# ehgus8/alpha-zero

Hardware: AMD Instinct MI355X
Metric: selfplay_games_per_sec (higher is better)
Workload: dtype bf16

## Files before the change

### alpha-zero_amd/azk/__init__.py

```python
import ctypes as C
import math
import os
import subprocess

import numpy as np

_HERE = os.path.dirname(os.path.abspath(__file__))
_CSRC = os.path.join(os.path.dirname(_HERE), "csrc")
LIB_PATH = os.path.join(_HERE, "libazk.so")

ABI_VERSION = 4
GAME_ID = {"tictactoe": 0, "connect4": 1, "gomoku": 2}
LEAF_F32, LEAF_BF16 = 0, 1
EMBED_POOL_COMPACT_MAX_SLOTS = 65279

SYMBOLS = [
    "azk_abi_version", "azk_last_error", "azk_create", "azk_destroy", "azk_geometry", "azk_reset_games",
    "azk_set_positions", "azk_begin_search", "azk_step_select", "azk_step_expand_backup", "azk_step",
    "azk_root_stats", "azk_root_children", "azk_export_tree", "azk_advance", "azk_get_positions",
    "azk_get_counters", "azk_reset_counters", "azk_check_device_error", "azk_gen_noise",
    "azk_rules_legal_moves", "azk_rules_legal_mask", "azk_rules_apply_move", "azk_rules_undo_move",
    "azk_rules_check_winner", "azk_rules_canonical", "azk_softmax_rows",
    "azk_step_tree", "azk_step_gather", "azk_recycle_finished", "azk_nn_patch_embed", "azk_nn_cls_attention", "azk_nn_patch_embed_scores", "azk_nn_cls_pool", "azk_debug_stamps", "azk_debug_stamps_raw", "azk_emit_finished", "azk_clear_cache", "azk_nn_heads_finalize", "azk_nn_layernorm_rows",
    "azk_vanilla_set_rng", "azk_vanilla_get_rng", "azk_vanilla_search", "azk_nn_embed_pool",
    "azk_nn_gemm_rows", "azk_nn_layernorm_sum", "azk_nn_heads_finalize_sum", "azk_nn_ln_heads",
    "azk_leaf_source_of", "azk_nn_embed_pool_leaves", "azk_nn_embed_pool_compact", "azk_nn_embed_pool_compact_leaves",
    "azk_nn_embed_fold", "azk_nn_embed_fold_leaves", "azk_nnx_embed_fold", "azk_nnx_embed_fold_leaves",
    "azk_nn_tail_gemm", "azk_nn_tail_gemm_lds", "azk_nn_tail_lds_footprint", "azk_nn_embed_fold_grid", "azk_nn_gemm_tok", "azk_nn_attention_tok", "azk_begin_search_budget", "azk_search_unfinished",
    "azk_nnx_embed_pool", "azk_nnx_embed_pool_leaves", "azk_nnx_gemm", "azk_nnx_gemm_h", "azk_nnx_gemm_h_lds",
    "azk_async_begin", "azk_async_step", "azk_async_drain", "azk_async_set_budget",
]


class AzkError(RuntimeError):
    pass


class Config(C.Structure):
    _fields_ = [("game", C.c_int32), ("rows", C.c_int32), ("cols", C.c_int32), ("n_games", C.c_int32),
                ("max_sims", C.c_int32), ("leaf_dtype", C.c_int32), ("device", C.c_int32),
                ("arena_nodes", C.c_int32), ("cache_entries", C.c_int32), ("cache_shared", C.c_int32), ("leaves_per_step", C.c_int32),
                ("tree_reuse", C.c_int32), ("reserved", C.c_int32 * 4)]


class LeafSource(C.Structure):
    _fields_ = [("leaf_flag", C.c_void_p), ("leaf_cells", C.c_void_p), ("to_move", C.c_void_p), ("leaf_depth", C.c_void_p),
                ("leaf_slot", C.c_void_p), ("n_leaf", C.c_void_p), ("n_games", C.c_int32), ("rows", C.c_int32), ("cols", C.c_int32),
                ("rc", C.c_int32), ("rc_pad", C.c_int32), ("planes", C.c_int32), ("flag_bytes", C.c_int32), ("cache_stamp", C.c_void_p)]


class EmbedPoolConsts(C.Structure):
    _fields_ = [("wt_frag", C.c_void_p), ("cpos_tok", C.c_void_p), ("score_tok", C.c_void_p), ("wconst_tok", C.c_void_p),
                ("xnconst_tok", C.c_void_p), ("z_all", C.c_void_p), ("l_all", C.c_void_p), ("score_msum", C.c_void_p),
                ("score_ref", C.c_void_p), ("num_heads", C.c_int32), ("ksize", C.c_int32), ("kp", C.c_int32),
                ("embed_dim", C.c_int32), ("ln_eps", C.c_float), ("work_stats", C.c_void_p)]


class EmbedFoldConsts(C.Structure):
    _fields_ = [("g_frag", C.c_void_p), ("e_frag", C.c_void_p), ("u2_tok", C.c_void_p), ("score_tok", C.c_void_p),
                ("wconst_tok", C.c_void_p), ("l_all", C.c_void_p), ("score_ref", C.c_void_p), ("inv_scales", C.c_void_p),
                ("num_heads", C.c_int32), ("ksize", C.c_int32), ("embed_dim", C.c_int32), ("ln_eps", C.c_float),
                ("work_stats", C.c_void_p)]


class TailGemm(C.Structure):
    _fields_ = [("a_bf16", C.c_void_p), ("lda", C.c_int32), ("a_batch_stride", C.c_int32), ("w_packed", C.c_void_p),
                ("m", C.c_int32), ("n_out", C.c_int32), ("k", C.c_int32), ("nbatch", C.c_int32), ("n_valid", C.c_void_p),
                ("bias", C.c_void_p), ("layernorm_a", C.c_int32), ("epilogue", C.c_int32), ("ln_eps", C.c_float),
                ("a_stats", C.c_void_p), ("a_stats_groups", C.c_int32), ("stats_out", C.c_void_p),
                ("out_bf16", C.c_void_p), ("ldo", C.c_int32), ("resid_bf16", C.c_void_p), ("ldr", C.c_int32),
                ("logits_out", C.c_void_p), ("values_out", C.c_void_p), ("action_dim", C.c_int32), ("a_col_sums", C.c_void_p)]


class GemmTok(C.Structure):
    _fields_ = [("a_bf16", C.c_void_p), ("lda", C.c_int32), ("w_packed", C.c_void_p), ("m", C.c_int32), ("n_out", C.c_int32), ("k", C.c_int32),
                ("n_valid", C.c_void_p), ("bias", C.c_void_p), ("epilogue", C.c_int32), ("out", C.c_void_p), ("ldo", C.c_int32),
                ("resid_bf16", C.c_void_p), ("ldr", C.c_int32)]


class EmbedPoolXConsts(C.Structure):
    _fields_ = [("wt_frag", C.c_void_p), ("cpos_tok", C.c_void_p), ("score_tok", C.c_void_p), ("wconst_tok", C.c_void_p),
                ("xnconst_tok", C.c_void_p), ("z_all", C.c_void_p), ("l_all", C.c_void_p), ("score_msum", C.c_void_p),
                ("score_ref", C.c_void_p), ("num_heads", C.c_int32), ("ksize", C.c_int32), ("kp", C.c_int32),
                ("embed_dim", C.c_int32), ("ln_eps", C.c_float), ("wt_scale", C.c_float), ("work_stats", C.c_void_p),
                ("wconst_h16_tok", C.c_void_p), ("pool_scale", C.c_float)]


class GemmX(C.Structure):
    _fields_ = [("a_f32", C.c_void_p), ("lda", C.c_int32), ("a_batch_stride", C.c_int32), ("w_packed", C.c_void_p),
                ("m", C.c_int32), ("n_out", C.c_int32), ("k", C.c_int32), ("nbatch", C.c_int32), ("n_valid", C.c_void_p),
                ("bias", C.c_void_p), ("layernorm_a", C.c_int32), ("epilogue", C.c_int32), ("ln_eps", C.c_float),
                ("a_stats", C.c_void_p), ("stats_out", C.c_void_p), ("out_f32", C.c_void_p), ("ldo", C.c_int32),
                ("resid_f32", C.c_void_p), ("ldr", C.c_int32), ("logits_out", C.c_void_p), ("values_out", C.c_void_p),
                ("action_dim", C.c_int32)]


class GemmH(C.Structure):
    _fields_ = [("a_hi", C.c_void_p), ("a_lo", C.c_void_p), ("a_f32", C.c_void_p), ("lda", C.c_int32), ("a_batch_stride", C.c_int32),
                ("w_packed", C.c_void_p), ("m", C.c_int32), ("n_out", C.c_int32), ("k", C.c_int32), ("nbatch", C.c_int32),
                ("n_valid", C.c_void_p), ("bias", C.c_void_p), ("col_sums", C.c_void_p), ("layernorm_a", C.c_int32), ("epilogue", C.c_int32),
                ("ln_eps", C.c_float), ("a_scale", C.c_float), ("w_scale", C.c_float), ("a_stats", C.c_void_p), ("stats_out", C.c_void_p),
                ("out_hi", C.c_void_p), ("out_lo", C.c_void_p), ("out_f32", C.c_void_p), ("ldo", C.c_int32), ("resid_f32", C.c_void_p),
                ("ldr", C.c_int32), ("logits_out", C.c_void_p), ("values_out", C.c_void_p), ("action_dim", C.c_int32), ("overflow_flag", C.c_void_p)]

# ... 64 lines not shown
    L.azk_clear_cache.argtypes = [vp, vp]
    L.azk_emit_finished.argtypes = [vp, vp, vp, vp, i64, vp, vp, vp]
    L.azk_debug_stamps.argtypes = [vp, vp]
    L.azk_check_device_error.argtypes = [vp, vp]
    L.azk_gen_noise.argtypes = [vp, u64, i64, i32, f64, vp, vp, vp]
    for name in ("azk_rules_legal_moves",):
        getattr(L, name).argtypes = [i32, i32, i32, vp, i32, vp, vp, vp]
    L.azk_rules_legal_mask.argtypes = [i32, i32, i32, vp, i32, vp, vp]
    L.azk_rules_apply_move.argtypes = [i32, i32, i32, vp, i32, vp, vp, vp, vp]
    L.azk_rules_undo_move.argtypes = [i32, i32, i32, vp, i32, vp, vp, vp]
    L.azk_rules_check_winner.argtypes = [i32, i32, i32, vp, i32, vp, vp, vp, vp]
    L.azk_rules_canonical.argtypes = [i32, i32, i32, vp, i32, vp, vp, vp]
    L.azk_softmax_rows.argtypes = [vp, i32, i32, vp, vp]
    L.azk_step_tree.argtypes = [vp, vp, vp, vp]
    L.azk_vanilla_set_rng.argtypes = [vp, i32, i32, vp, vp]
    L.azk_vanilla_get_rng.argtypes = [vp, i32, i32, vp, vp]
    L.azk_vanilla_search.argtypes = [vp, i32, vp]
    L.azk_step_gather.argtypes = [vp, vp, vp, vp]
    L.azk_recycle_finished.argtypes = [vp, vp, vp]
    L.azk_nn_patch_embed_scores.argtypes = [vp, i32, vp, vp, vp, vp, vp, vp, vp, vp, i32, i32, i32, i32, i32, i32, i32, i32, C.c_float, vp, vp]
    L.azk_nn_embed_pool.argtypes = [vp, i32, vp, vp, vp, vp, vp, vp, i32, i32, i32, i32, i32, i32, i32, i32, C.c_float, vp, vp]
    L.azk_leaf_source_of.argtypes = [vp, vp, C.POINTER(LeafSource)]
    L.azk_nn_embed_pool_leaves.argtypes = [C.POINTER(LeafSource), vp, vp, vp, vp, vp, vp, i32, i32, i32, i32, C.c_float, vp]
    L.azk_nn_embed_pool_compact.argtypes = [vp, i32, C.POINTER(EmbedPoolConsts), vp, i32, i32, i32, i32, vp, vp, vp]
    L.azk_nn_embed_pool_compact_leaves.argtypes = [C.POINTER(LeafSource), C.POINTER(EmbedPoolConsts), vp, vp, vp]
    L.azk_nn_embed_fold.argtypes = [vp, i32, C.POINTER(EmbedFoldConsts), vp, i32, i32, i32, i32, vp, vp, vp]
    L.azk_nn_embed_fold_leaves.argtypes = [C.POINTER(LeafSource), C.POINTER(EmbedFoldConsts), vp, vp, vp]
    L.azk_nnx_embed_fold.argtypes = [vp, i32, C.POINTER(EmbedFoldConsts), vp, i32, i32, i32, i32, vp, vp, vp]
    L.azk_nnx_embed_fold_leaves.argtypes = [C.POINTER(LeafSource), C.POINTER(EmbedFoldConsts), vp, vp, vp]
    L.azk_begin_search_budget.argtypes = [vp, vp, i32, i32, vp]
    L.azk_search_unfinished.argtypes = [vp, vp, vp]
    L.azk_nn_tail_gemm.argtypes = [C.POINTER(TailGemm), vp]
    L.azk_nn_tail_gemm_lds.argtypes = [C.POINTER(TailGemm), vp]
    L.azk_nn_gemm_tok.argtypes = [C.POINTER(GemmTok), vp]
    L.azk_nn_attention_tok.argtypes = [vp, vp, i32, i32, i32, i32, vp, vp]
    L.azk_nnx_embed_pool.argtypes = [vp, i32, C.POINTER(EmbedPoolXConsts), vp, i32, i32, i32, i32, vp, vp, vp]
    L.azk_nnx_embed_pool_leaves.argtypes = [C.POINTER(LeafSource), C.POINTER(EmbedPoolXConsts), vp, vp, vp]
    L.azk_nnx_gemm.argtypes = [C.POINTER(GemmX), vp]
    L.azk_nnx_gemm_h.argtypes = [C.POINTER(GemmH), vp]
    L.azk_nnx_gemm_h_lds.argtypes = [C.POINTER(GemmH), vp]
    L.azk_async_begin.argtypes = [vp, C.POINTER(AsyncConfig), vp]
    L.azk_async_step.argtypes = [vp, vp, vp, i32, vp]
    L.azk_async_set_budget.argtypes = [vp, i32, i32, vp]
    L.azk_async_drain.argtypes = [vp, vp, vp, vp, i64, vp, vp]
    L.azk_nn_ln_heads.argtypes = [vp, vp, vp, C.c_float, vp, vp, i32, i32, i32, i32, vp, vp, vp, vp]
    L.azk_nn_gemm_rows.argtypes = [vp, i32, vp, i32, i32, i32, i32, vp, vp, vp, vp, vp]
    L.azk_nn_layernorm_sum.argtypes = [vp, i32, i32, vp, vp, vp, vp, C.c_float, vp, vp, vp, i32, i32, vp, vp]
    L.azk_nn_heads_finalize_sum.argtypes = [vp, i32, i32, i32, vp, i32, i32, vp, vp, vp, vp]
    L.azk_nn_layernorm_rows.argtypes = [vp, vp, vp, C.c_float, vp, vp, i32, i32, vp, vp]
    L.azk_nn_heads_finalize.argtypes = [vp, i32, i32, i32, vp, vp, vp, vp]
    L.azk_nn_cls_pool.argtypes = [vp, vp, vp, vp, i32, i32, i32, i32, vp, vp]
    L.azk_nn_cls_attention.argtypes = [vp, vp, vp, i32, vp, i32, i32, i32, i32, vp]
    L.azk_nn_patch_embed.argtypes = [vp, i32, vp, vp, vp, vp, vp, vp, i32, i32, i32, i32, i32, i32, i32, C.c_float, vp]
    for name in SYMBOLS:
        f = getattr(L, name)
        if name not in ("azk_last_error", "azk_destroy"):
            f.restype = i32
    _LIB = L
    return L


def _torch():
    import torch
    if not torch.cuda.is_available():
        raise AzkError("no GPU visible: the azk engine runs only on an MI355X (no CPU fallback)")
    return torch
# ... 672 lines not shown

def nn_tail_gemm(a, w_packed, n_out, k, epilogue=TAIL_BF16, nbatch=1, a_batch_stride=0, bias=None, out=None, resid=None,
                 a_stats=None, stats_out=None, logits=None, values=None, action_dim=0, count=None, eps=1e-5, col_sums=None, lds=False):
    torch = _torch()
    assert a.dtype == torch.bfloat16 and a.stride(-1) == 1 and a.dim() == 2
    d = TailGemm()
    d.a_bf16, d.lda, d.a_batch_stride, d.w_packed = a.data_ptr(), a.stride(0), int(a_batch_stride), w_packed.data_ptr()
    d.m, d.n_out, d.k, d.nbatch = a.shape[0], int(n_out), int(k), int(nbatch)
    d.n_valid = count.data_ptr() if count is not None else None
    d.bias = bias.data_ptr() if bias is not None else None
    d.layernorm_a, d.epilogue, d.ln_eps = (1 if a_stats is not None else 0), int(epilogue), float(eps)
    if a_stats is not None:
        assert a_stats.dtype == torch.float32 and a_stats.dim() == 3 and a_stats.shape[2] == 2 and a_stats.is_contiguous()
        d.a_stats, d.a_stats_groups = a_stats.data_ptr(), a_stats.shape[1]
    if stats_out is not None:
        assert stats_out.dtype == torch.float32 and tuple(stats_out.shape) == (a.shape[0], nbatch * n_out // 64, 2) and stats_out.is_contiguous()
        d.stats_out = stats_out.data_ptr()
    if out is not None:
        assert out.dtype == torch.bfloat16 and out.stride(-1) == 1
        d.out_bf16, d.ldo = out.data_ptr(), out.stride(0)
    if resid is not None:
        d.resid_bf16, d.ldr = resid.data_ptr(), resid.stride(0)
    if logits is not None:
        assert logits.dtype == torch.float32 and values.dtype == torch.float32 and logits.is_contiguous()
        d.logits_out, d.values_out, d.action_dim = logits.data_ptr(), values.data_ptr(), int(action_dim)
    if col_sums is not None:
        assert col_sums.dtype == torch.float32 and col_sums.is_contiguous() and col_sums.numel() >= nbatch * n_out
        d.a_col_sums = col_sums.data_ptr()
    rc = (lib().azk_nn_tail_gemm_lds if lds else lib().azk_nn_tail_gemm)(C.byref(d), _stream())
    if rc != 0:
        raise AzkError(f"azk_nn_tail_gemm{'_lds' if lds else ''} failed ({rc})")


TOK_BF16, TOK_GELU, TOK_RESID, TOK_F32 = 0, 1, 2, 4


def pack_linear_weight128(w):
    torch = _torch()
    n_out, k = w.shape
    npad = (n_out + 127) // 128 * 128
    wp = torch.zeros(npad, k, dtype=torch.float32, device=w.device)
    wp[:n_out] = w.float()
    return pack_linear_weight(wp)


def nn_gemm_tok(a, w_packed, n_out, epilogue=TOK_BF16, bias=None, out=None, resid=None, count=None):
    torch = _torch()
    assert a.dtype == torch.bfloat16 and a.dim() == 2 and a.stride(1) == 1 and n_out % 128 == 0
    m, k = a.shape
    if out is None:
        out = torch.empty((m, n_out), dtype=torch.float32 if epilogue == TOK_F32 else torch.bfloat16, device=a.device)
    assert out.stride(1) == 1 and out.dtype == (torch.float32 if epilogue == TOK_F32 else torch.bfloat16)
    d = GemmTok()
    d.a_bf16, d.lda, d.w_packed, d.m, d.n_out, d.k = a.data_ptr(), a.stride(0), w_packed.data_ptr(), m, int(n_out), k
    d.n_valid = count.data_ptr() if count is not None else None
    if bias is not None:
        assert bias.dtype == torch.float32 and bias.numel() >= n_out
        d.bias = bias.data_ptr()
    d.epilogue, d.out, d.ldo = int(epilogue), out.data_ptr(), out.stride(0)
    if resid is not None:
        assert resid.dtype == torch.bfloat16 and resid.stride(1) == 1
        d.resid_bf16, d.ldr = resid.data_ptr(), resid.stride(0)
    rc = lib().azk_nn_gemm_tok(C.byref(d), _stream())
    if rc != 0:
        raise AzkError(f"azk_nn_gemm_tok failed ({rc})")
    return out
# ... 352 lines not shown
```

### alpha-zero_amd/csrc/azk_nn.hip

```cpp
#include <hip/hip_runtime.h>
#include <hip/hip_bf16.h>
#include <stdint.h>
#include <stdio.h>
#include <stdlib.h>
#include <string.h>
#include <type_traits>

#include "azk.h"
#include "azk_launch.h"
#include "azk_tail_common.h"

namespace {

typedef __attribute__((ext_vector_type(8))) __bf16 bf16x8;
typedef __attribute__((ext_vector_type(4))) float f32x4;

struct EmbedArgs {
    const void *boards;
    int boards_f32;
    const __hip_bfloat16 *wt;
    const float *cpos;
    const float *ln_w, *ln_b;
    __hip_bfloat16 *x;
    __hip_bfloat16 *xhat;
// ... 2540 lines not shown
        uint2 rr[EPI == TAIL_EPI_RESID ? RT : 1][4];
        if (EPI == TAIL_EPI_RESID) {
#pragma unroll
            for (int i = 0; i < RT; i++)
#pragma unroll
                for (int j = 0; j < 4; j++) rr[i][j] = *(const uint2 *)(a.resid + (size_t)min(row0 + 16 * i + 4 * l4 + j, a.M - 1) * a.ldr + col0);
        }
        if (EPI == TAIL_EPI_HEADS) {
            f32x4 hv[RT][4];
#pragma unroll
            for (int i = 0; i < RT; i++)
#pragma unroll
                for (int j = 0; j < 4; j++) {
                    hv[i][j] = f32x4{acc[i][0][j] + bv[0], acc[i][1][j] + bv[1], acc[i][2][j] + bv[2], acc[i][3][j] + bv[3]};
#pragma unroll
                    for (int c = 0; c < 4; c++)
                        if (col0 + c == a.action_dim) hv[i][j][c] = tanhf(hv[i][j][c]);
                }
#pragma unroll
            for (int i = 0; i < RT; i++)
#pragma unroll
                for (int j = 0; j < 4; j++) {
                    const int row = row0 + 16 * i + 4 * l4 + j;
#pragma unroll
                    for (int c = 0; c < 4; c++) {
                        const int col = col0 + c;
                        if (row < nvalid && col < a.action_dim) a.logits[(size_t)row * a.action_dim + col] = hv[i][j][c];
                        if (row < nvalid && col == a.action_dim) a.values[row] = hv[i][j][c];
                    }
                }
        } else {
            uint2 o[RT][4];
            f32x2 ps[RT][4];
#pragma unroll
            for (int i = 0; i < RT; i++)
#pragma unroll
                for (int j = 0; j < 4; j++) {
                    f32x4 v = {acc[i][0][j] + bv[0], acc[i][1][j] + bv[1], acc[i][2][j] + bv[2], acc[i][3][j] + bv[3]};
                    if (EPI == TAIL_EPI_GELU) {
#pragma unroll
                        for (int c = 0; c < 4; c++) v[c] = gelu_erf(v[c]);
                    }
                    if (EPI == TAIL_EPI_RESID) {
                        v[0] += __uint_as_float(rr[i][j].x << 16); v[1] += __uint_as_float(rr[i][j].x & 0xffff0000u);
                        v[2] += __uint_as_float(rr[i][j].y << 16); v[3] += __uint_as_float(rr[i][j].y & 0xffff0000u);
                    }
                    union { bf16x4 b4; uint2 u; } ob;
                    ob.b4 = __builtin_convertvector(v, bf16x4);
                    o[i][j] = ob.u;
                    if (a.stats_out) {
                        const f32x4 vr = __builtin_convertvector(ob.b4, f32x4);
                        ps[i][j] = f32x2{row16_sum((vr[0] + vr[1]) + (vr[2] + vr[3])),
                                         row16_sum((vr[0] * vr[0] + vr[1] * vr[1]) + (vr[2] * vr[2] + vr[3] * vr[3]))};
                    }
                }
            const int ngr = a.nbatch * (a.N >> 6), gr = b * (a.N >> 6) + g;
#pragma unroll
            for (int i = 0; i < RT; i++)
#pragma unroll
                for (int j = 0; j < 4; j++) {
                    const int row = row0 + 16 * i + 4 * l4 + j;
                    if (row < nvalid) *(uint2 *)(a.out + (size_t)row * a.ldo + col0) = o[i][j];
                    if (a.stats_out && l15 == 0 && row < nvalid) *(f32x2 *)(a.stats_out + ((size_t)row * ngr + gr) * 2) = ps[i][j];
                }
        }
    }
}

template <int RTLO, int RTHI, int KCH, int AMODE, int EPI, int NWR, int NWC, int NWK>
__global__ __launch_bounds__(64 * NWR * NWC * NWK, 1) void k_tail_gemm(TailArgs a) {
    __shared__ f32x4 kred[NWK > 1 ? (NWK - 1) * RTHI * 4 * 64 : 1];
    asm volatile("" :: "s"(a.A), "s"(a.Wp), "s"(a.out), "s"(a.bias), "s"(a.resid), "s"(a.stats_in), "s"(a.stats_out), "s"(a.logits), "s"(a.values),
                 "s"(a.lda), "s"(a.ldo), "s"(a.N), "s"(a.nbatch), "s"(a.wave_slots), "s"(a.M), "s"(a.a_batch), "s"(a.w_batch), "s"(a.ldr),
                 "s"(a.ln_eps), "s"(a.action_dim));
    const int nvalid = a.count ? min(a.M, *a.count) : a.M;
    const int strip_waves = (a.N >> 6) * a.nbatch * NWK;
    int rt = RTLO;
    while (rt < RTHI && ((nvalid + 16 * rt * NWR - 1) / (16 * rt * NWR)) * NWR * strip_waves > a.wave_slots) rt++;
    if (RTHI >= RTLO + 2 && rt == RTLO + 2) tail_items<(RTHI >= RTLO + 2 ? RTLO + 2 : RTLO), KCH, AMODE, EPI, NWR, NWC, NWK>(a, nvalid, kred);
    else if (RTHI >= RTLO + 1 && rt == RTLO + 1) tail_items<(RTHI >= RTLO + 1 ? RTLO + 1 : RTLO), KCH, AMODE, EPI, NWR, NWC, NWK>(a, nvalid, kred);
    else tail_items<RTLO, KCH, AMODE, EPI, NWR, NWC, NWK>(a, nvalid, kred);
}

int tail_cu_count() {
    static int cus = 0;
    if (!cus) {
        int dev = 0;
        if (hipGetDevice(&dev) != hipSuccess || hipDeviceGetAttribute(&cus, hipDeviceAttributeMultiprocessorCount, dev) != hipSuccess || cus <= 0) cus = 256;
    }
    return cus;
}

template <int RTLO, int RTHI, int KCH, int AMODE, int EPI, int NWR, int NWC, int NWK = 1>
int launch_tail(TailArgs &a, hipStream_t st) {
    static_assert(RTHI <= RTLO + 2, "three tile heights per kernel");
    static int slots = 0;
    if (!slots) {
        int nb = 0;
        if (hipOccupancyMaxActiveBlocksPerMultiprocessor(&nb, k_tail_gemm<RTLO, RTHI, KCH, AMODE, EPI, NWR, NWC, NWK>, 64 * NWR * NWC * NWK, 0) != hipSuccess || nb < 1) nb = 1;
        slots = nb * NWR * NWC * NWK * tail_cu_count();
    }
    a.wave_slots = slots;
    const long long items = (long long)((a.M + 16 * RTLO * NWR - 1) / (16 * RTLO * NWR)) * (a.N / (64 * NWC)) * a.nbatch;
    const unsigned blocks = (unsigned)(items < 8192 ? items : 8192);
    k_tail_gemm<RTLO, RTHI, KCH, AMODE, EPI, NWR, NWC, NWK><<<blocks, 64 * NWR * NWC * NWK, 0, st>>>(a);
    return hipGetLastError() == hipSuccess ? AZK_OK : AZK_ERR_HIP;
}
}

extern "C" int32_t azk_nn_tail_gemm(const azk_tail_gemm *t, void *stream) {
    if (!t || !t->a_bf16 || !t->w_packed || t->m < 0 || t->n_out < 64 || (t->n_out & 63) || t->nbatch < 1) return AZK_ERR_ARG;
    if ((t->k != 512 && t->k != 2048 && t->k != 384) || t->lda < t->k || (t->lda & 7) || (t->a_batch_stride & 7)) return AZK_ERR_ARG;
    if (t->epilogue < 0 || t->epilogue > 3 || (t->layernorm_a && (t->k != 512 || !t->a_stats || t->a_stats_groups != 8))) return AZK_ERR_ARG;
    if (t->epilogue == TAIL_EPI_HEADS ? (!t->logits_out || !t->values_out || t->action_dim + 1 > t->n_out * t->nbatch) : (!t->out_bf16 || t->ldo < t->n_out * t->nbatch || (t->ldo & 3)))
        return AZK_ERR_ARG;
    if (t->epilogue == TAIL_EPI_RESID && (!t->resid_bf16 || (t->ldr & 3))) return AZK_ERR_ARG;
    if (t->m == 0) return AZK_OK;
    TailArgs a = {};
    a.A = (const unsigned short *)t->a_bf16; a.lda = t->lda; a.a_batch = t->a_batch_stride; a.Wp = (const uint4 *)t->w_packed;
    a.w_batch = (long long)(t->n_out / 64) * (t->k / 32) * 4 * 64;
    a.M = t->m; a.N = t->n_out; a.nbatch = t->nbatch; a.count = t->n_valid; a.bias = t->bias; a.out = (unsigned short *)t->out_bf16; a.ldo = t->ldo;
    a.resid = (const unsigned short *)t->resid_bf16; a.ldr = t->ldr; a.ln_eps = t->ln_eps; a.logits = t->logits_out; a.values = t->values_out;
    a.action_dim = t->action_dim; a.stats_in = t->a_stats; a.stats_groups = t->a_stats_groups; a.stats_out = t->stats_out;
    hipStream_t st = (hipStream_t)stream;
    const bool wide = t->n_out % 128 == 0 && t->n_out >= 1024;
    if (t->k == 384)
        return !t->layernorm_a && t->epilogue == TAIL_EPI_BF16 ? launch_tail<2, 2, 3, 0, TAIL_EPI_BF16, 1, 1, 4>(a, st) : AZK_ERR_ARG;
    if (t->k == 512) {
        if (t->layernorm_a) {
            if (t->epilogue == TAIL_EPI_GELU) return wide ? launch_tail<2, 4, 16, 1, TAIL_EPI_GELU, 2, 2>(a, st) : launch_tail<2, 2, 16, 1, TAIL_EPI_GELU, 1, 1>(a, st);
            if (t->epilogue == TAIL_EPI_HEADS) return launch_tail<1, 1, 4, 1, TAIL_EPI_HEADS, 1, 1, 4>(a, st);
            if (t->epilogue == TAIL_EPI_BF16) return launch_tail<2, 2, 16, 1, TAIL_EPI_BF16, 1, 1>(a, st);
            return AZK_ERR_ARG;
        }
        if (t->epilogue == TAIL_EPI_BF16) return launch_tail<2, 2, 4, 0, TAIL_EPI_BF16, 1, 1, 4>(a, st);
        if (t->epilogue == TAIL_EPI_GELU) return wide ? launch_tail<2, 4, 16, 0, TAIL_EPI_GELU, 2, 2>(a, st) : launch_tail<2, 2, 16, 0, TAIL_EPI_GELU, 1, 1>(a, st);
        if (t->epilogue == TAIL_EPI_RESID) return launch_tail<2, 2, 16, 0, TAIL_EPI_RESID, 1, 1>(a, st);
        return launch_tail<2, 2, 16, 0, TAIL_EPI_HEADS, 1, 1>(a, st);
    }
    if (t->epilogue == TAIL_EPI_RESID) return launch_tail<2, 4, 16, 0, TAIL_EPI_RESID, 1, 1, 4>(a, st);
    if (t->epilogue == TAIL_EPI_BF16) return launch_tail<2, 4, 16, 0, TAIL_EPI_BF16, 1, 1, 4>(a, st);
    return AZK_ERR_ARG;
}
```

### alpha-zero_amd/csrc/azk_tail_common.h

```cpp
#pragma once
#include <hip/hip_runtime.h>
#include <stdint.h>

namespace azk_tail {

typedef __attribute__((ext_vector_type(8))) __bf16 bf16x8;
typedef __attribute__((ext_vector_type(4))) __bf16 bf16x4;
typedef __attribute__((ext_vector_type(4))) float f32x4;
typedef __attribute__((ext_vector_type(2))) float f32x2;

struct TailArgs {
    const unsigned short *A; int lda, a_batch;
    const uint4 *Wp; long long w_batch;
    int M, N, nbatch;
    const int *count;
    const float *bias;
    unsigned short *out; int ldo;
    const unsigned short *resid; int ldr;
    float ln_eps;
    const float *stats_in; int stats_groups;
    float *stats_out;
    float *logits, *values; int action_dim;
    int wave_slots;
    const float *csum;
};

enum { TAIL_EPI_BF16 = 0, TAIL_EPI_GELU = 1, TAIL_EPI_RESID = 2, TAIL_EPI_HEADS = 3 };

__device__ __forceinline__ float gelu_erf(float x) {
    const float z = fabsf(x) * 0.70710678118654752f;
    const float t = __builtin_amdgcn_rcpf(1.0f + 0.3275911f * z);
    const float poly = t * (0.254829592f + t * (-0.284496736f + t * (1.421413741f + t * (-1.453152027f + t * 1.061405429f))));
    const float erf_abs = 1.0f - poly * __expf(-z * z);
    return 0.5f * x * (1.0f + copysignf(erf_abs, x));
}

__device__ __forceinline__ float row16_sum(float v) {
    v += __builtin_bit_cast(float, __builtin_amdgcn_update_dpp(0, __builtin_bit_cast(int, v), 0xB1, 0xF, 0xF, true));
    v += __builtin_bit_cast(float, __builtin_amdgcn_update_dpp(0, __builtin_bit_cast(int, v), 0x4E, 0xF, 0xF, true));
    v += __builtin_bit_cast(float, __builtin_amdgcn_update_dpp(0, __builtin_bit_cast(int, v), 0x141, 0xF, 0xF, true));
    v += __builtin_bit_cast(float, __builtin_amdgcn_update_dpp(0, __builtin_bit_cast(int, v), 0x140, 0xF, 0xF, true));
    return v;
}

__device__ __forceinline__ float quad_sum(float v) {
    v += __builtin_bit_cast(float, __builtin_amdgcn_update_dpp(0, __builtin_bit_cast(int, v), 0xB1, 0xF, 0xF, true));
    v += __builtin_bit_cast(float, __builtin_amdgcn_update_dpp(0, __builtin_bit_cast(int, v), 0x4E, 0xF, 0xF, true));
    return v;
}

}
```

### alpha-zero_amd/pvnet.py

```python
import math

import torch
import torch.nn.functional as F


class NetConfig:
    def __init__(self, rows, cols, channels, action_dim, patch_size=5, embed_dim=512, num_heads=8, depth=1, dropout=0.0):
        self.rows, self.cols, self.channels, self.action_dim = rows, cols, channels, action_dim
        self.patch_size, self.embed_dim, self.num_heads, self.depth = patch_size, embed_dim, num_heads, depth
        self.dropout = dropout

    @property
    def tokens(self):
        return self.rows * self.cols + 1

    def flops_full(self):
        T, D, A, C, k = self.tokens, self.embed_dim, self.action_dim, self.channels, self.patch_size
        conv = 2 * (T - 1) * D * C * k * k
        blk = 2 * T * D * 3 * D + 2 * 2 * T * T * D + 2 * T * D * D + 2 * 2 * T * D * 4 * D
        return conv + self.depth * blk + 2 * D * (A + 1)

    def flops_cls(self):
        T, D, A, C, k = self.tokens, self.embed_dim, self.action_dim, self.channels, self.patch_size
        conv = 2 * (T - 1) * D * C * k * k
# ... 70 lines not shown
        for k_ in dst:
            _copy_into(dst[k_], src[k_])
    elif isinstance(dst, (list, tuple)):
        for d_, s_ in zip(dst, src):
            _copy_into(d_, s_)
    elif hasattr(dst, "t") and isinstance(getattr(dst, "t"), dict):
        _copy_into(dst.t, src.t)


class PolicyValueNet:

    def __init__(self, cfg, weights=None, seed=0, device="cpu", dtype=torch.float32, path="cls"):
        self.cfg = cfg
        w = weights if weights is not None else init_weights(cfg, seed)
        want = reference_key_shapes(cfg)
        if set(w) != set(want):
            raise KeyError(f"state_dict keys differ: missing {sorted(set(want) - set(w))}, unexpected {sorted(set(w) - set(want))}")
        for k_, shp in want.items():
            if tuple(w[k_].shape) != tuple(shp):
                raise ValueError(f"{k_}: shape {tuple(w[k_].shape)} != {shp}")
        self.master = {k_: torch.as_tensor(v).detach().to(torch.float32).cpu().clone() for k_, v in w.items()}
        self.path = path
        self.fast_outputs = False
        self.last_value_pre_tanh = False
        self.out_buffers = None
        self.hip_tail = False
        self.use_hip_tail = False
        self.leaf_source = None
        self.fuse_ln_heads = True
        self.fused_embed_pool = False
        self.chain_tail = False
        self.use_chain_tail = True
        self.use_lds_tail = True
        self._tail_ws = {}
        self._tail_ws_retired = []
        self._compact = None
        self.use_compact = True
        self._foldu = None
        self.use_fold_u = True
        self._scheds = {}
        self.kernel_timers = None
        self.live_count = None
        self.to(device, dtype)

    def state_dict(self):
        return {k_: v.clone() for k_, v in self.master.items()}

    @classmethod
    def from_state_dict(cls, cfg, sd, **kw):
        return cls(cfg, weights=sd, **kw)

    def load_state_dict(self, sd, in_place=True):
        want = reference_key_shapes(self.cfg)
        for k_, shape in want.items():
            assert k_ in sd and tuple(sd[k_].shape) == tuple(shape), k_
        names = ("w", "_hip", "_fold", "_compact", "_exact", "_foldu", "_blocks")
        old = {n_: getattr(self, n_, None) for n_ in names}
        old_flags = (self.fused_embed_pool, self.chain_tail, self.hip_tail, self._gelu_epilogue)
        self.master = {k_: torch.as_tensor(sd[k_]).detach().to("cpu", torch.float32).clone() for k_ in want}
        self.to(self.device, self.dtype)
        if not in_place:
            return False
        new = {n_: getattr(self, n_, None) for n_ in names}
        if old_flags != (self.fused_embed_pool, self.chain_tail, self.hip_tail, self._gelu_epilogue) or not _same_structure(old, new):
            return False
        _copy_into(old, new)
# ... 550 lines not shown
        azk.nn_gemm_rows(hh, f["W3P"], D, ksplit=4, partials=P3, count=cnt)
        y = torch.empty((n, D), **bf)
        azk.nn_layernorm_sum(P3, f["lnf_w"], f["lnf_b"], y, resid=x1b, count=cnt)
        Np = f["bh_f"].numel()
        P4 = torch.empty((4, n, Np), dtype=torch.float32, device=dev)
        azk.nn_gemm_rows(y, f["WhP"], Np, ksplit=4, partials=P4, count=cnt)
        if self.out_buffers is not None:
            lb, vb = self.out_buffers
        else:
            lb = torch.empty((n, A), dtype=torch.float32, device=dev)
            vb = torch.empty(n, dtype=torch.float32, device=dev)
        azk.nn_heads_finalize_sum(P4, f["bh_f"], A, lb, vb, count=cnt)
        return lb, (vb if self.out_buffers is not None else vb[:, None])

    def tail_chain(self, z):
        import azk
        cfg, f = self.cfg, self._fold
        n, A, D, H = z.shape[0], cfg.action_dim, cfg.embed_dim, cfg.num_heads
        dev, cnt = z.device, self.live_count
        key = id(self.leaf_source) if self.leaf_source is not None else None
        ws = self._tail_ws.get(key)
        if ws is None or ws["rows"] < n:
            rows = n if ws is None else max(n, 2 * ws["rows"])
            if ws is not None:
                self._tail_ws_retired.append(ws)
            bf = dict(dtype=torch.bfloat16, device=dev)
            ws = dict(rows=rows, u=torch.empty((rows, D), **bf), x1=torch.empty((rows, D), **bf), hh=torch.empty((rows, 4 * D), **bf),
                      x2=torch.empty((rows, D), **bf), st1=torch.empty((rows, D // 64, 2), dtype=torch.float32, device=dev),
                      st2=torch.empty((rows, D // 64, 2), dtype=torch.float32, device=dev))
            self._tail_ws[key] = ws
        ws = {k_: (v[:n] if k_ != "rows" else v) for k_, v in ws.items()}
        if z.shape[-1] == azk.EMBED_FOLD_ROW:
            kf = azk.EMBED_FOLD_ROW
            self._launch(azk.nn_tail_gemm, z.view(n, H * kf), self._foldu.weight, D // H, kf, azk.TAIL_BF16, nbatch=H, a_batch_stride=kf, out=ws["u"], count=cnt)
        else:
            self._launch(azk.nn_tail_gemm, z.view(n, H * D), f["WvHP"], D // H, D, azk.TAIL_BF16, nbatch=H, a_batch_stride=D, out=ws["u"], count=cnt)
        self._launch(azk.nn_tail_gemm, ws["u"], f["WoP"], D, D, azk.TAIL_BF16, bias=f["bias1_f"], out=ws["x1"], stats_out=ws["st1"], count=cnt)
        lds = getattr(self, "use_lds_tail", True)
        self._launch(azk.nn_tail_gemm, ws["x1"], f["W0GP"], 4 * D, D, azk.TAIL_GELU, bias=f["b0G_f"], out=ws["hh"], a_stats=ws["st1"], count=cnt,
                     col_sums=f["W0GP_csum"] if lds else None, lds=lds)
        self._launch(azk.nn_tail_gemm, ws["hh"], f["W3P"], D, 4 * D, azk.TAIL_RESID, bias=f["b3_f"], resid=ws["x1"], out=ws["x2"], stats_out=ws["st2"], count=cnt,
                     lds=lds)
        if self.out_buffers is not None:
            lb, vb = self.out_buffers
        else:
            lb = torch.empty((n, A), dtype=torch.float32, device=dev)
            vb = torch.empty(n, dtype=torch.float32, device=dev)
        self._launch(azk.nn_tail_gemm, ws["x2"], f["WhGP"], f["bhG_f"].numel(), D, azk.TAIL_HEADS, bias=f["bhG_f"], a_stats=ws["st2"], logits=lb, values=vb,
                         action_dim=A, count=cnt)
        return lb, (vb if self.out_buffers is not None else vb[:, None])

    def tail_fast(self, z):
        kt = self.kernel_timers[-1] if self.kernel_timers is not None and len(self.kernel_timers) >= (2 if self.fused_embed_pool else 3) else None
        self._tail_timer = kt
        try:
            if kt is None or z.dtype == torch.float32 or (getattr(self, "chain_tail", False) and self.use_chain_tail):
                return self._tail_fast(z)
            kt.start()
            out = self._tail_fast(z)
            kt.stop()
            return out
        finally:
            self._tail_timer = None

    def _launch(self, fn, *args, **kw):
        kt = getattr(self, "_tail_timer", None)
        if kt is not None:
            kt.start()
        fn(*args, **kw)
        if kt is not None:
# ... 247 lines not shown
```

### include/azk.h

```cpp
#ifndef AZK_H
#define AZK_H

#include <stdint.h>

#ifdef __cplusplus
extern "C" {
#endif

#define AZK_ABI_VERSION 4

#define AZK_TICTACTOE 0
#define AZK_CONNECT4 1
#define AZK_GOMOKU 2

#define AZK_LEAF_F32 0
#define AZK_LEAF_BF16 1

#define AZK_OK 0
#define AZK_ERR_ARG (-1)
#define AZK_ERR_HIP (-2)
#define AZK_ERR_ARENA_FULL (-3)
#define AZK_ERR_STATE (-4)

typedef struct azk_engine azk_engine;
// ... 159 lines not shown
    int32_t num_heads, ksize, kp, embed_dim;
    float ln_eps;
    uint64_t *work_stats;
} azk_embed_pool_consts;
int32_t azk_nn_embed_pool_compact(const void *boards_dev, int32_t boards_are_f32, const azk_embed_pool_consts *consts,
                                  void *z_out_bf16_dev, int32_t n, int32_t channels, int32_t rows, int32_t cols,
                                  const int32_t *n_valid_dev, int32_t *sched_dev, void *stream);
#define AZK_EMBED_POOL_COMPACT_MAX_SLOTS 65279
int32_t azk_nn_embed_pool_compact_leaves(const azk_leaf_source *src, const azk_embed_pool_consts *consts, void *z_out_bf16_dev,
                                         int32_t *sched_dev, void *stream);

int32_t azk_nn_gemm_rows(const void *a_bf16_dev, int32_t lda, const void *w_packed_dev, int32_t m, int32_t n_out, int32_t k,
                         int32_t ksplit, float *partials_out_dev, const float *bias_dev, void *gelu_out_bf16_dev,
                         const int32_t *n_valid_dev, void *stream);
typedef struct azk_tail_gemm {
    const void *a_bf16; int32_t lda, a_batch_stride;
    const void *w_packed;
    int32_t m, n_out, k, nbatch;
    const int32_t *n_valid;
    const float *bias;
    int32_t layernorm_a, epilogue;
    float ln_eps;
    const float *a_stats; int32_t a_stats_groups;
    float *stats_out;
    void *out_bf16; int32_t ldo;
    const void *resid_bf16; int32_t ldr;
    float *logits_out, *values_out; int32_t action_dim;
    const float *a_col_sums;
} azk_tail_gemm;
int32_t azk_nn_tail_gemm(const azk_tail_gemm *desc, void *stream);
int32_t azk_nn_tail_gemm_lds(const azk_tail_gemm *desc, void *stream);
int32_t azk_nn_tail_lds_footprint(int32_t small);
int32_t azk_nn_embed_fold_grid(int32_t max_workgroups);

int32_t azk_nn_ln_heads(const void *x_bf16_dev, const float *ln_w_dev, const float *ln_b_dev, float eps, const void *w_packed_dev,
                        const float *bias_dev, int32_t n, int32_t embed_dim, int32_t n_out_padded, int32_t action_dim,
                        float *logits_out_dev, float *values_out_dev, const int32_t *n_valid_dev, void *stream);
int32_t azk_nn_layernorm_sum(const float *partials_dev, int32_t nsplit, int32_t m_stride, const float *bias_dev,
                             const void *resid_bf16_dev, const float *w_dev, const float *b_dev, float eps, void *y_bf16_dev,
                             const float *add_bias_dev, void *x_out_bf16_dev, int32_t n, int32_t embed_dim,
                             const int32_t *n_valid_dev, void *stream);
int32_t azk_nn_heads_finalize_sum(const float *partials_dev, int32_t nsplit, int32_t m_stride, int32_t ld, const float *bias_dev,
                                  int32_t action_dim, int32_t n, float *logits_out_dev, float *values_out_dev,
                                  const int32_t *n_valid_dev, void *stream);

#define AZK_EMBED_FOLD_ROW 384
#define AZK_EMBED_FOLD_MAX_SLOTS 8192
typedef struct azk_embed_fold_consts {
    const void *g_frag, *e_frag;
    const float *u2_tok, *score_tok, *wconst_tok, *l_all, *score_ref;
    const float *inv_scales;
    int32_t num_heads, ksize, embed_dim;
    float ln_eps;
    uint64_t *work_stats;
} azk_embed_fold_consts;
int32_t azk_nn_embed_fold(const void *boards_dev, int32_t boards_are_f32, const azk_embed_fold_consts *consts, void *rows_out_bf16_dev,
                          int32_t n, int32_t channels, int32_t rows, int32_t cols, const int32_t *n_valid_dev, int32_t *sched_dev,
                          void *stream);
int32_t azk_nn_embed_fold_leaves(const azk_leaf_source *src, const azk_embed_fold_consts *consts, void *rows_out_bf16_dev,
                                 int32_t *sched_dev, void *stream);
int32_t azk_nnx_embed_fold(const void *boards_dev, int32_t boards_are_f32, const azk_embed_fold_consts *consts, float *rows_out_f32_dev,
                           int32_t n, int32_t channels, int32_t rows, int32_t cols, const int32_t *n_valid_dev, int32_t *sched_dev,
                           void *stream);
int32_t azk_nnx_embed_fold_leaves(const azk_leaf_source *src, const azk_embed_fold_consts *consts, float *rows_out_f32_dev,
                                  int32_t *sched_dev, void *stream);

// ... 82 lines not shown
```

Measured before the change: 1021.

## Fuse per-head fold-U GEMM and output projection into one tail kernel

After: 967.4. 0.947x the previous value.

```diff
diff --git a/alpha-zero_amd/azk/__init__.py b/alpha-zero_amd/azk/__init__.py
--- a/alpha-zero_amd/azk/__init__.py
+++ b/alpha-zero_amd/azk/__init__.py
@@ -26,7 +26,7 @@
     "azk_nn_gemm_rows", "azk_nn_layernorm_sum", "azk_nn_heads_finalize_sum", "azk_nn_ln_heads",
     "azk_leaf_source_of", "azk_nn_embed_pool_leaves", "azk_nn_embed_pool_compact", "azk_nn_embed_pool_compact_leaves",
     "azk_nn_embed_fold", "azk_nn_embed_fold_leaves", "azk_nnx_embed_fold", "azk_nnx_embed_fold_leaves",
-    "azk_nn_tail_gemm", "azk_nn_tail_gemm_lds", "azk_nn_tail_lds_footprint", "azk_nn_embed_fold_grid", "azk_nn_gemm_tok", "azk_nn_attention_tok", "azk_begin_search_budget", "azk_search_unfinished",
+    "azk_nn_tail_gemm", "azk_nn_tail_gemm_lds", "azk_nn_tail_vo", "azk_nn_tail_lds_footprint", "azk_nn_embed_fold_grid", "azk_nn_gemm_tok", "azk_nn_attention_tok", "azk_begin_search_budget", "azk_search_unfinished",
     "azk_nnx_embed_pool", "azk_nnx_embed_pool_leaves", "azk_nnx_gemm", "azk_nnx_gemm_h", "azk_nnx_gemm_h_lds",
     "azk_async_begin", "azk_async_step", "azk_async_drain", "azk_async_set_budget",
 ]
@@ -70,6 +70,12 @@
                 ("a_stats", C.c_void_p), ("a_stats_groups", C.c_int32), ("stats_out", C.c_void_p),
                 ("out_bf16", C.c_void_p), ("ldo", C.c_int32), ("resid_bf16", C.c_void_p), ("ldr", C.c_int32),
                 ("logits_out", C.c_void_p), ("values_out", C.c_void_p), ("action_dim", C.c_int32), ("a_col_sums", C.c_void_p)]
+
+
+class TailVo(C.Structure):
+    _fields_ = [("z_bf16", C.c_void_p), ("ldz", C.c_int32), ("m", C.c_int32), ("k", C.c_int32), ("heads", C.c_int32), ("head_dim", C.c_int32),
+                ("wf_packed", C.c_void_p), ("wo_packed", C.c_void_p), ("bias", C.c_void_p), ("n_valid", C.c_void_p),
+                ("out_bf16", C.c_void_p), ("ldo", C.c_int32), ("stats_out", C.c_void_p)]
 
 
 class GemmTok(C.Structure):
@@ -200,6 +206,7 @@
     L.azk_search_unfinished.argtypes = [vp, vp, vp]
     L.azk_nn_tail_gemm.argtypes = [C.POINTER(TailGemm), vp]
     L.azk_nn_tail_gemm_lds.argtypes = [C.POINTER(TailGemm), vp]
+    L.azk_nn_tail_vo.argtypes = [C.POINTER(TailVo), vp]
     L.azk_nn_gemm_tok.argtypes = [C.POINTER(GemmTok), vp]
     L.azk_nn_attention_tok.argtypes = [vp, vp, i32, i32, i32, i32, vp, vp]
     L.azk_nnx_embed_pool.argtypes = [vp, i32, C.POINTER(EmbedPoolXConsts), vp, i32, i32, i32, i32, vp, vp, vp]
@@ -938,6 +945,24 @@
         raise AzkError(f"azk_nn_tail_gemm{'_lds' if lds else ''} failed ({rc})")
 
 
+def nn_tail_vo(z, wf_packed, wo_packed, heads, head_dim, bias=None, out=None, stats_out=None, count=None):
+    torch = _torch()
+    assert z.dtype == torch.bfloat16 and z.stride(-1) == 1 and z.dim() == 2
+    assert out is not None and out.dtype == torch.bfloat16 and out.stride(-1) == 1 and out.shape[0] == z.shape[0]
+    d = TailVo()
+    d.z_bf16, d.ldz, d.m, d.k, d.heads, d.head_dim = z.data_ptr(), z.stride(0), z.shape[0], z.shape[1] // int(heads), int(heads), int(head_dim)
+    d.wf_packed, d.wo_packed = wf_packed.data_ptr(), wo_packed.data_ptr()
+    d.bias = bias.data_ptr() if bias is not None else None
+    d.n_valid = count.data_ptr() if count is not None else None
+    d.out_bf16, d.ldo = out.data_ptr(), out.stride(0)
+    if stats_out is not None:
+        assert stats_out.dtype == torch.float32 and tuple(stats_out.shape) == (z.shape[0], heads * head_dim // 64, 2) and stats_out.is_contiguous()
+        d.stats_out = stats_out.data_ptr()
+    rc = lib().azk_nn_tail_vo(C.byref(d), _stream())
+    if rc != 0:
+        raise AzkError(f"azk_nn_tail_vo failed ({rc})")
+
+
 TOK_BF16, TOK_GELU, TOK_RESID, TOK_F32 = 0, 1, 2, 4
 
 
diff --git a/alpha-zero_amd/csrc/azk_nn.hip b/alpha-zero_amd/csrc/azk_nn.hip
--- a/alpha-zero_amd/csrc/azk_nn.hip
+++ b/alpha-zero_amd/csrc/azk_nn.hip
@@ -2596,37 +2596,8 @@
         } else {
             uint2 o[RT][4];
             f32x2 ps[RT][4];
-#pragma unroll
-            for (int i = 0; i < RT; i++)
-#pragma unroll
-                for (int j = 0; j < 4; j++) {
-                    f32x4 v = {acc[i][0][j] + bv[0], acc[i][1][j] + bv[1], acc[i][2][j] + bv[2], acc[i][3][j] + bv[3]};
-                    if (EPI == TAIL_EPI_GELU) {
-#pragma unroll
-                        for (int c = 0; c < 4; c++) v[c] = gelu_erf(v[c]);
-                    }
-                    if (EPI == TAIL_EPI_RESID) {
-                        v[0] += __uint_as_float(rr[i][j].x << 16); v[1] += __uint_as_float(rr[i][j].x & 0xffff0000u);
-                        v[2] += __uint_as_float(rr[i][j].y << 16); v[3] += __uint_as_float(rr[i][j].y & 0xffff0000u);
-                    }
-                    union { bf16x4 b4; uint2 u; } ob;
-                    ob.b4 = __builtin_convertvector(v, bf16x4);
-                    o[i][j] = ob.u;
-                    if (a.stats_out) {
-                        const f32x4 vr = __builtin_convertvector(ob.b4, f32x4);
-                        ps[i][j] = f32x2{row16_sum((vr[0] + vr[1]) + (vr[2] + vr[3])),
-                                         row16_sum((vr[0] * vr[0] + vr[1] * vr[1]) + (vr[2] * vr[2] + vr[3] * vr[3]))};
-                    }
-                }
-            const int ngr = a.nbatch * (a.N >> 6), gr = b * (a.N >> 6) + g;
-#pragma unroll
-            for (int i = 0; i < RT; i++)
-#pragma unroll
-                for (int j = 0; j < 4; j++) {
-                    const int row = row0 + 16 * i + 4 * l4 + j;
-                    if (row < nvalid) *(uint2 *)(a.out + (size_t)row * a.ldo + col0) = o[i][j];
-                    if (a.stats_out && l15 == 0 && row < nvalid) *(f32x2 *)(a.stats_out + ((size_t)row * ngr + gr) * 2) = ps[i][j];
-                }
+            azk_tail::tail_epi_rows<RT, EPI>(acc, bv, rr, a.stats_out != nullptr, o, ps);
+            azk_tail::tail_epi_store<RT>(o, ps, a.out, a.ldo, col0, a.stats_out, a.nbatch * (a.N >> 6), b * (a.N >> 6) + g, row0, nvalid);
         }
     }
 }
@@ -2668,6 +2639,142 @@
     const long long items = (long long)((a.M + 16 * RTLO * NWR - 1) / (16 * RTLO * NWR)) * (a.N / (64 * NWC)) * a.nbatch;
     const unsigned blocks = (unsigned)(items < 8192 ? items : 8192);
     k_tail_gemm<RTLO, RTHI, KCH, AMODE, EPI, NWR, NWC, NWK><<<blocks, 64 * NWR * NWC * NWK, 0, st>>>(a);
+    return hipGetLastError() == hipSuccess ? AZK_OK : AZK_ERR_HIP;
+}
+
+struct TailVoArgs {
+    const unsigned short *Z; int ldz;
+    const uint4 *Wf, *Wo;
+    const float *bias; const int *count;
+    unsigned short *out; int ldo; float *stats_out;
+    int M, wg_slots;
+};
+
+template <int RT, int NK>
+__device__ __forceinline__ void tail_vo_tile(const TailVoArgs &a, const int nvalid, f32x4 *sh) {
+    static_assert(NK >= 4 && NK <= 24, "ring depth");
+    const int lane = threadIdx.x & 63, wave = threadIdx.x >> 6, l15 = lane & 15, l4 = lane >> 4;
+    const int rtiles = (nvalid + 16 * RT - 1) / (16 * RT);
+    const int ct = (blockIdx.x >> 3) & 7, rt = (blockIdx.x & 7) + 8 * (blockIdx.x >> 6);
+    if (rt >= rtiles) return;
+    const int row0 = rt * 16 * RT;
+    union BF { uint4 u; bf16x8 v; };
+    const int wv = __builtin_amdgcn_readfirstlane(wave);
+    const unsigned short *zt = a.Z + (size_t)row0 * a.ldz + 768 * wv;
+    unsigned zo[RT];
+#pragma unroll
+    for (int i = 0; i < RT; i++) zo[i] = (unsigned)min(16 * i + l15, nvalid - 1 - row0) * (unsigned)a.ldz + 8u * l4;
+    const uint4 *bp1 = a.Wf + (size_t)wv * (2 * 12 * 4 * 64);
+    const uint4 *bp2 = a.Wo + ((size_t)ct * 16 + 4 * wv) * 4 * 64;
+    const unsigned ul = lane;
+    const int col0 = 64 * ct + 4 * l15;
+    f32x4 bv = {0.f, 0.f, 0.f, 0.f};
+    BF af[NK][RT], bf[NK][4], b2[4][4];
+#pragma unroll
+    for (int g = 0; g < NK; g++) {
+        const uint4 *pb = bp1 + 256 * g;
+        asm volatile("" : "+s"(pb));
+#pragma unroll
+        for (int i = 0; i < RT; i++) af[g][i].u = *(const uint4 *)(zt + 32 * g + zo[i]);
+#pragma unroll
+        for (int c = 0; c < 4; c++) bf[g][c].u = pb[ul + 64 * c];
+    }
+    __builtin_amdgcn_sched_barrier(0);
+    unsigned char *ush = (unsigned char *)(sh + wave * RT * 4 * 64);
+    f32x4 tot[RT][4], p[RT][4];
+#pragma unroll
+    for (int g = 0; g < 24; g++) {
+        const int sl = g % NK, s = g % 3, q = (g / 3) & 3, hh = g / 12;
+#pragma unroll
+        for (int i = 0; i < RT; i++)
+#pragma unroll
+            for (int c = 0; c < 4; c++)
+                p[i][c] = __builtin_amdgcn_mfma_f32_16x16x32_bf16(af[sl][i].v, bf[sl][c].v, s == 0 ? f32x4{0.f, 0.f, 0.f, 0.f} : p[i][c], 0, 0, 0);
+        __builtin_amdgcn_sched_barrier(0);
+        if (g + NK < 24) {
+            const uint4 *pb = bp1 + 256 * (g + NK);
+            asm volatile("" : "+s"(pb));
+#pragma unroll
+            for (int i = 0; i < RT; i++) af[sl][i].u = *(const uint4 *)(zt + 32 * (g + NK) + zo[i]);
+#pragma unroll
+            for (int c = 0; c < 4; c++) bf[sl][c].u = pb[ul + 64 * c];
+        } else if (g + NK < 28) {
+            const uint4 *pb = bp2 + 256 * (g + NK - 24);
+            asm volatile("" : "+s"(pb));
+#pragma unroll
+            for (int c = 0; c < 4; c++) b2[g + NK - 24][c].u = pb[ul + 64 * c];
+            if (g + NK == 27 && a.bias) bv = *(const f32x4 *)(a.bias + col0);
+        }
+        __builtin_amdgcn_sched_barrier(0);
+        if (s < 2) continue;
+#pragma unroll
+        for (int i = 0; i < RT; i++)
+#pragma unroll
+            for (int c = 0; c < 4; c++) tot[i][c] = q == 0 ? p[i][c] : tot[i][c] + p[i][c];
+        if (q == 3) {
+            uint2 o[RT][4];
+            f32x2 ps[RT][4];
+            azk_tail::tail_epi_rows<RT, TAIL_EPI_BF16>(tot, f32x4{0.f, 0.f, 0.f, 0.f}, nullptr, false, o, ps);
+#pragma unroll
+            for (int i = 0; i < RT; i++)
+#pragma unroll
+                for (int j = 0; j < 4; j++)
+                    *(uint2 *)(ush + (16 * i + 4 * l4 + j) * 256 + (((8 * hh + (l15 >> 1)) ^ (4 * l4 + j)) << 4) + 8 * (l15 & 1)) = o[i][j];
+        }
+    }
+    __builtin_amdgcn_fence(__ATOMIC_RELEASE, "wavefront");
+    __builtin_amdgcn_wave_barrier();
+    __builtin_amdgcn_fence(__ATOMIC_ACQUIRE, "wavefront");
+    BF a2[RT][4];
+#pragma unroll
+    for (int s = 0; s < 4; s++)
+#pragma unroll
+        for (int i = 0; i < RT; i++) a2[i][s].u = *(const uint4 *)(ush + (16 * i + l15) * 256 + (((4 * s + l4) ^ l15) << 4));
+    f32x4 acc[RT][4];
+#pragma unroll
+    for (int i = 0; i < RT; i++)
+#pragma unroll
+        for (int c = 0; c < 4; c++) acc[i][c] = f32x4{0.f, 0.f, 0.f, 0.f};
+#pragma unroll
+    for (int s = 0; s < 4; s++)
+#pragma unroll
+        for (int i = 0; i < RT; i++)
+#pragma unroll
+            for (int c = 0; c < 4; c++) acc[i][c] = __builtin_amdgcn_mfma_f32_16x16x32_bf16(a2[i][s].v, b2[s][c].v, acc[i][c], 0, 0, 0);
+    if (wave > 0) {
+#pragma unroll
+        for (int i = 0; i < RT; i++)
+#pragma unroll
+            for (int c = 0; c < 4; c++) sh[(wave * RT * 4 + i * 4 + c) * 64 + lane] = acc[i][c];
+    }
+    __syncthreads();
+    if (wave > 0) return;
+#pragma unroll
+    for (int w = 1; w < 4; w++)
+#pragma unroll
+        for (int i = 0; i < RT; i++)
+#pragma unroll
+            for (int c = 0; c < 4; c++) acc[i][c] += sh[(w * RT * 4 + i * 4 + c) * 64 + lane];
+    uint2 o[RT][4];
+    f32x2 ps[RT][4];
+    azk_tail::tail_epi_rows<RT, TAIL_EPI_BF16>(acc, bv, nullptr, a.stats_out != nullptr, o, ps);
+    azk_tail::tail_epi_store<RT>(o, ps, a.out, a.ldo, col0, a.stats_out, 8, ct, row0, nvalid);
+}
+
+template <int NK1, int NK2, int NK4>
+__global__ __launch_bounds__(256, 1) void k_tail_vo(TailVoArgs a) {
+    __shared__ f32x4 sh[4 * 4 * 4 * 64];
+    asm volatile("" :: "s"(a.Z), "s"(a.Wf), "s"(a.Wo), "s"(a.bias), "s"(a.out), "s"(a.stats_out), "s"(a.ldz), "s"(a.ldo), "s"(a.M), "s"(a.wg_slots));
+    const int nvalid = a.count ? min(a.M, *a.count) : a.M;
+    if (((nvalid + 15) >> 4) * 8 <= a.wg_slots) tail_vo_tile<1, NK1>(a, nvalid, sh);
+    else if (((nvalid + 31) >> 5) * 8 <= a.wg_slots) tail_vo_tile<2, NK2>(a, nvalid, sh);
+    else tail_vo_tile<4, NK4>(a, nvalid, sh);
+}
+
+int launch_tail_vo(TailVoArgs &a, hipStream_t st) {
+    a.wg_slots = tail_cu_count();
+    const unsigned blocks = (unsigned)((((a.M + 15) / 16 + 7) / 8) * 64);
+    k_tail_vo<12, 12, 6><<<blocks, 256, 0, st>>>(a);
     return hipGetLastError() == hipSuccess ? AZK_OK : AZK_ERR_HIP;
 }
 }
@@ -2706,3 +2813,14 @@
     if (t->epilogue == TAIL_EPI_BF16) return launch_tail<2, 4, 16, 0, TAIL_EPI_BF16, 1, 1, 4>(a, st);
     return AZK_ERR_ARG;
 }
+
+extern "C" int32_t azk_nn_tail_vo(const azk_tail_vo *t, void *stream) {
+    if (!t || !t->z_bf16 || !t->wf_packed || !t->wo_packed || !t->out_bf16 || t->m < 0) return AZK_ERR_ARG;
+    if (t->k != AZK_EMBED_FOLD_ROW || t->head_dim != 64 || t->heads != 8) return AZK_ERR_ARG;
+    if (t->ldz < t->heads * t->k || (t->ldz & 7) || t->ldo < t->heads * t->head_dim || (t->ldo & 3)) return AZK_ERR_ARG;
+    if (t->m == 0) return AZK_OK;
+    TailVoArgs a = {};
+    a.Z = (const unsigned short *)t->z_bf16; a.ldz = t->ldz; a.Wf = (const uint4 *)t->wf_packed; a.Wo = (const uint4 *)t->wo_packed;
+    a.bias = t->bias; a.count = t->n_valid; a.out = (unsigned short *)t->out_bf16; a.ldo = t->ldo; a.stats_out = t->stats_out; a.M = t->m;
+    return launch_tail_vo(a, (hipStream_t)stream);
+}
diff --git a/alpha-zero_amd/csrc/azk_tail_common.h b/alpha-zero_amd/csrc/azk_tail_common.h
--- a/alpha-zero_amd/csrc/azk_tail_common.h
+++ b/alpha-zero_amd/csrc/azk_tail_common.h
@@ -49,4 +49,46 @@
     return v;
 }
 
+template <int RT, int EPI>
+__device__ __forceinline__ void tail_epi_rows(const f32x4 (&acc)[RT][4], const f32x4 bv, const uint2 (*rr)[4], const bool stats,
+                                              uint2 (&o)[RT][4], f32x2 (&ps)[RT][4]) {
+#pragma unroll
+    for (int i = 0; i < RT; i++)
+#pragma unroll
+        for (int j = 0; j < 4; j++) {
+            f32x4 v = {acc[i][0][j] + bv[0], acc[i][1][j] + bv[1], acc[i][2][j] + bv[2], acc[i][3][j] + bv[3]};
+            if (EPI == TAIL_EPI_GELU) {
+#pragma unroll
+                for (int c = 0; c < 4; c++) v[c] = gelu_erf(v[c]);
+            }
+            if (EPI == TAIL_EPI_RESID) {
+                v[0] += __uint_as_float(rr[i][j].x << 16); v[1] += __uint_as_float(rr[i][j].x & 0xffff0000u);
+                v[2] += __uint_as_float(rr[i][j].y << 16); v[3] += __uint_as_float(rr[i][j].y & 0xffff0000u);
+            }
+            union { bf16x4 b4; uint2 u; } ob;
+            ob.b4 = __builtin_convertvector(v, bf16x4);
+            o[i][j] = ob.u;
+            if (stats) {
+                const f32x4 vr = __builtin_convertvector(ob.b4, f32x4);
+                ps[i][j] = f32x2{row16_sum((vr[0] + vr[1]) + (vr[2] + vr[3])),
+                                 row16_sum((vr[0] * vr[0] + vr[1] * vr[1]) + (vr[2] * vr[2] + vr[3] * vr[3]))};
+            }
+        }
 }
+
+template <int RT>
+__device__ __forceinline__ void tail_epi_store(const uint2 (&o)[RT][4], const f32x2 (&ps)[RT][4], unsigned short *out, const int ldo,
+                                               const int col0, float *stats_out, const int ngr, const int gr, const int row0,
+                                               const int nvalid) {
+    const int l15 = threadIdx.x & 15, l4 = (threadIdx.x & 63) >> 4;
+#pragma unroll
+    for (int i = 0; i < RT; i++)
+#pragma unroll
+        for (int j = 0; j < 4; j++) {
+            const int row = row0 + 16 * i + 4 * l4 + j;
+            if (row < nvalid) *(uint2 *)(out + (size_t)row * ldo + col0) = o[i][j];
+            if (stats_out && l15 == 0 && row < nvalid) *(f32x2 *)(stats_out + ((size_t)row * ngr + gr) * 2) = ps[i][j];
+        }
+}
+
+}
diff --git a/alpha-zero_amd/pvnet.py b/alpha-zero_amd/pvnet.py
--- a/alpha-zero_amd/pvnet.py
+++ b/alpha-zero_amd/pvnet.py
@@ -126,6 +126,7 @@
         self.chain_tail = False
         self.use_chain_tail = True
         self.use_lds_tail = True
+        self.use_fused_vo = True
         self._tail_ws = {}
         self._tail_ws_retired = []
         self._compact = None
@@ -742,10 +743,18 @@
         ws = {k_: (v[:n] if k_ != "rows" else v) for k_, v in ws.items()}
         if z.shape[-1] == azk.EMBED_FOLD_ROW:
             kf = azk.EMBED_FOLD_ROW
-            self._launch(azk.nn_tail_gemm, z.view(n, H * kf), self._foldu.weight, D // H, kf, azk.TAIL_BF16, nbatch=H, a_batch_stride=kf, out=ws["u"], count=cnt)
+            fused_vo = getattr(self, "use_fused_vo", True) and D == 512 and H == 8
+            if fused_vo:
+                self._launch(azk.nn_tail_vo, z.view(n, H * kf), self._foldu.weight, f["WoP"], H, D // H, bias=f["bias1_f"], out=ws["x1"], stats_out=ws["st1"],
+                             count=cnt)
+                self._launch(lambda: None)
+            else:
+                self._launch(azk.nn_tail_gemm, z.view(n, H * kf), self._foldu.weight, D // H, kf, azk.TAIL_BF16, nbatch=H, a_batch_stride=kf, out=ws["u"], count=cnt)
         else:
+            fused_vo = False
             self._launch(azk.nn_tail_gemm, z.view(n, H * D), f["WvHP"], D // H, D, azk.TAIL_BF16, nbatch=H, a_batch_stride=D, out=ws["u"], count=cnt)
-        self._launch(azk.nn_tail_gemm, ws["u"], f["WoP"], D, D, azk.TAIL_BF16, bias=f["bias1_f"], out=ws["x1"], stats_out=ws["st1"], count=cnt)
+        if not fused_vo:
+            self._launch(azk.nn_tail_gemm, ws["u"], f["WoP"], D, D, azk.TAIL_BF16, bias=f["bias1_f"], out=ws["x1"], stats_out=ws["st1"], count=cnt)
         lds = getattr(self, "use_lds_tail", True)
         self._launch(azk.nn_tail_gemm, ws["x1"], f["W0GP"], 4 * D, D, azk.TAIL_GELU, bias=f["b0G_f"], out=ws["hh"], a_stats=ws["st1"], count=cnt,
                      col_sums=f["W0GP_csum"] if lds else None, lds=lds)
diff --git a/include/azk.h b/include/azk.h
--- a/include/azk.h
+++ b/include/azk.h
@@ -215,6 +215,16 @@
 int32_t azk_nn_tail_gemm_lds(const azk_tail_gemm *desc, void *stream);
 int32_t azk_nn_tail_lds_footprint(int32_t small);
 int32_t azk_nn_embed_fold_grid(int32_t max_workgroups);
+typedef struct azk_tail_vo {
+    const void *z_bf16; int32_t ldz;
+    int32_t m, k, heads, head_dim;
+    const void *wf_packed, *wo_packed;
+    const float *bias;
+    const int32_t *n_valid;
+    void *out_bf16; int32_t ldo;
+    float *stats_out;
+} azk_tail_vo;
+int32_t azk_nn_tail_vo(const azk_tail_vo *desc, void *stream);
 
 int32_t azk_nn_ln_heads(const void *x_bf16_dev, const float *ln_w_dev, const float *ln_b_dev, float eps, const void *w_packed_dev,
                         const float *bias_dev, int32_t n, int32_t embed_dim, int32_t n_out_padded, int32_t action_dim,
```
